# domanovi/FEC_Erasure_Code_Unit_Test_Relay

Measured on AMD Instinct MI355X. Metric: GiB/s device-resident erasure encode+decode, 300B pkts, T=10; %HBM roofline, higher is better.
Workload: dtype u8; 1 GPU; encode 1000010 + decode 1000000 x 300B packets per GPU, one stream per GPU, (T,B,N)=(10,3,3); T=10, B=3, N=3, packets_per_gpu=1000000

## Files before the change

### fec_erasure_code_unit_test_relay_amd/_lib.py

```python
from __future__ import annotations

import ctypes
import os

_HERE = os.path.dirname(os.path.abspath(__file__))
LIB_PATH = os.environ.get("FEC_AMD_LIB") or os.path.join(_HERE, "libfec_amd.so")
HEADER_PATHS = [os.path.join(_HERE, "..", "include", "fec_amd.h")]

FEC_OK = 0
FEC_ERR_ARG = -1
FEC_ERR_HIP = -2
FEC_ERR_NOMEM = -3
FEC_ERR_WORKSPACE = -4
FEC_ERR_SEQUENCE = -5
FEC_ERR_HISTORY = -6

KERNEL_NAMES = ["fec_encode_kernel", "fec_scan_kernel", "fec_plan_kernel", "fec_copy_kernel",
                "fec_recover_kernel"]


class FecError(RuntimeError):
    def __init__(self, status: int, what: str = ""):
        msg = lib().fec_strerror(status).decode() if _lib is not None else str(status)
        if status == FEC_ERR_HIP and _lib is not None:
# ... 4 lines not shown
        self.status = status


_lib = None


def lib() -> ctypes.CDLL:
    global _lib
    if _lib is not None:
        return _lib
    if not os.path.exists(LIB_PATH):
        raise RuntimeError(
            f"{LIB_PATH} is missing: the HIP extension must be built first "
            "(make -C fec_erasure_code_unit_test_relay_amd/csrc); there is no fallback")
    try:
        import torch
    except ImportError:
        pass
    L = ctypes.CDLL(LIB_PATH)
    vp, i32, i64 = ctypes.c_void_p, ctypes.c_int, ctypes.c_int64
    ip = ctypes.POINTER(ctypes.c_int)
    i64p = ctypes.POINTER(ctypes.c_int64)
    L.fec_strerror.restype = ctypes.c_char_p
    L.fec_strerror.argtypes = [i32]
    L.fec_last_error.restype = i32
    L.fec_last_error.argtypes = [ctypes.c_char_p, ctypes.c_size_t]
    L.fec_version.restype = i32
    L.fec_codec_create.argtypes = [i32, i32, i32, i32, ctypes.POINTER(vp)]
    L.fec_codec_destroy.argtypes = [vp]
    L.fec_codec_geometry.argtypes = [vp, ip, ip, ip, ip]
    L.fec_codec_generator.argtypes = [vp, vp]
    L.fec_codec_set_encode_path.argtypes = [vp, i32]
    L.fec_encode_tile_fetch.argtypes = [i32, i32, i32, i32, i32, ip, ip, ip, ip]
    L.fec_codec_set_copy_path.argtypes = [vp, i32]
    L.fec_codec_set_plan_path.argtypes = [vp, i32]
    L.fec_codec_info.argtypes = [vp, ctypes.c_char_p, ctypes.c_size_t]
    L.fec_codec_set_episode_dedup.argtypes = [vp, i32]
    L.fec_debug_stamps.argtypes = [vp, i32, vp]
    L.fec_encode_batch.argtypes = [vp, vp, vp, i64, i64, vp, vp, vp]
    L.fec_decode_workspace_bytes.restype = ctypes.c_size_t
    L.fec_decode_workspace_bytes.argtypes = [vp, i64]
    L.fec_decode_batch.argtypes = [vp, vp, vp, i64, vp, vp, vp, ctypes.c_size_t, vp]
    L.fec_decode_counters.argtypes = [vp, i64p, i64p, i64p]
    L.fec_streams_create.argtypes = [i32, i32, i32, i32, i32, ctypes.POINTER(vp)]
    L.fec_streams_destroy.argtypes = [vp]
    L.fec_streams_encode.argtypes = [vp, vp, i32, vp, vp, vp, vp, vp]
    L.fec_streams_decode.argtypes = [vp, vp, i32, vp, vp, vp, vp, vp]
    L.fec_streams_state.argtypes = [vp, i32, i64p, i64p]
    L.fec_streams_encode_burst.argtypes = [vp, vp, vp, i32, vp, vp, vp, vp, vp]
    L.fec_streams_decode_burst.argtypes = [vp, vp, vp, i32, vp, vp, vp, vp, vp]
    L.fec_streams_plan_burst_host.argtypes = [i32, i32, i32, i32, vp, vp, i32, vp]
    L.fec_streams_create_mixed.argtypes = [i32, vp, i32, vp, i32, ctypes.POINTER(vp)]
    L.fec_streams_codes.argtypes = [vp, ip, ip]
    L.fec_streams_stream_geometry.argtypes = [vp, i32, ip, ip, ip, ip, ip, ip]
    L.fec_streams_set_code.argtypes = [vp, i32, i32]
    L.fec_streams_mixed_fit.argtypes = [i32, vp, i32, vp, vp, vp, vp]
    L.fec_decode_stream_create.argtypes = [ctypes.POINTER(vp)]
    L.fec_decode_stream_destroy.argtypes = [vp]
    L.fec_decode_stream_state.argtypes = [vp, i64p, i64p]
    L.fec_decode_stream_push.argtypes = [vp, vp, vp, vp, vp, i64, i64, vp, vp, i64p, vp, ctypes.c_size_t, vp]
    L.fec_decode_plan_stats.argtypes = [vp, i64p, i64p]
    L.fec_decode_plan.argtypes = [vp, vp, i64, vp, ctypes.c_size_t, vp]
    L.fec_decode_apply.argtypes = [vp, vp, vp, i64, vp, vp, vp, ctypes.c_size_t, vp]
    L.fec_decode_copy.argtypes = [vp, vp, vp, i64, vp, vp, vp]
    L.fec_decode_recover.argtypes = [vp, vp, i64, vp, vp, vp, ctypes.c_size_t, vp]
    L.fec_timing_enable.argtypes = [vp, i32]
# ... 45 lines not shown
    L.fec_relay_streams_plan_host.argtypes = [i32, i32, vp, vp, i32, vp, vp]
    L.fec_sdswdf_create.argtypes = [i32, i32, i32, i32, i32, i32, ctypes.POINTER(vp)]
    L.fec_sdswdf_destroy.argtypes = [vp]
    L.fec_sdswdf_geometry.argtypes = [vp, ip, ip, ip, ip, ip, ip, ip]
    L.fec_sdswdf_tile_geometry.argtypes = [i32, i32, i32, i32, i32, i32, i64, ip, ip]
    L.fec_sdswdf_relay_batch.argtypes = [vp, vp, i64, vp, i64, vp, vp]
    L.fec_sdswdf_destination_batch.argtypes = [vp, vp, vp, i64, vp, vp, vp]
    L.fec_sdswdf_relay_plan.argtypes = [vp, vp, i64, vp, vp, i64, i64p, ip]
    L.fec_sdswdf_dest_plan.argtypes = [vp, vp, vp, i64, vp, vp, vp, i64, i64p, ip]
    L.fec_sdswdf_relay_batch_starts.argtypes = [vp, vp, i64, vp, i64, vp, i32, vp, vp]
    L.fec_sdswdf_destination_batch_starts.argtypes = [vp, vp, vp, i64, vp, i32, vp, vp, vp]
    L.fec_relay_vr_create.argtypes = [i32, i32, vp, i32, i64, ctypes.POINTER(vp)]
    L.fec_relay_vr_destroy.argtypes = [vp]
    L.fec_relay_vr_geometry.argtypes = [vp, ip, ip, ip]
    L.fec_relay_vr_run.argtypes = [vp, vp, vp, vp, vp, vp, vp, vp, vp]
    L.fec_relay_session_create.argtypes = [i32, i32, i64, vp, i64, vp, i64, ctypes.POINTER(vp)]
    L.fec_relay_session_destroy.argtypes = [vp]
    L.fec_relay_session_info.argtypes = [vp, vp, vp]
    L.fec_relay_session_relay_offsets.argtypes = [vp, vp]
    L.fec_relay_session_hop1_headers.argtypes = [vp, vp]
    L.fec_relay_session_dest_meta.argtypes = [vp, vp, vp]
    L.fec_relay_session_run.argtypes = [vp, vp, vp, vp, vp, vp, vp]
    L.fec_relay_session_hop1.argtypes = [vp, vp, i64, vp, vp]
    for name in ["fec_relay_session_create", "fec_relay_session_destroy", "fec_relay_session_info",
                 "fec_relay_session_relay_offsets", "fec_relay_session_hop1_headers", "fec_relay_session_dest_meta",
                 "fec_relay_session_run", "fec_relay_session_hop1", "fec_sdswdf_create", "fec_sdswdf_destroy", "fec_sdswdf_geometry", "fec_sdswdf_tile_geometry", "fec_sdswdf_relay_batch",
                 "fec_sdswdf_destination_batch", "fec_sdswdf_relay_plan", "fec_sdswdf_dest_plan",
                 "fec_sdswdf_relay_batch_starts", "fec_sdswdf_destination_batch_starts", "fec_relay_vr_create",
                 "fec_relay_vr_destroy", "fec_relay_vr_geometry", "fec_relay_vr_run",
                 "fec_swdf_create", "fec_swdf_destroy", "fec_swdf_geometry", "fec_swdf_relay_batch",
                 "fec_swdf_destination_batch", "fec_relay_streams_create", "fec_relay_streams_destroy",
                 "fec_relay_streams_geometry", "fec_relay_streams_relay", "fec_relay_streams_destination",
                 "fec_relay_streams_state", "fec_relay_streams_fit", "fec_relay_streams_plan_host", "fec_codec_create", "fec_codec_destroy", "fec_codec_set_encode_path",
                 "fec_encode_tile_fetch", "fec_codec_set_copy_path", "fec_codec_set_plan_path", "fec_codec_info", "fec_codec_set_episode_dedup", "fec_debug_stamps", "fec_codec_geometry",
                 "fec_codec_generator", "fec_encode_batch", "fec_decode_batch", "fec_decode_plan",
                 "fec_decode_stream_create", "fec_decode_stream_destroy", "fec_decode_stream_state",
                 "fec_decode_stream_push", "fec_streams_create", "fec_streams_destroy", "fec_streams_encode",
                 "fec_streams_decode", "fec_streams_state", "fec_streams_encode_burst",
                 "fec_streams_decode_burst", "fec_streams_plan_burst_host", "fec_streams_create_mixed",
                 "fec_streams_codes", "fec_streams_stream_geometry", "fec_streams_set_code",
                 "fec_streams_mixed_fit",
                 "fec_decode_apply", "fec_decode_copy", "fec_decode_recover",
                 "fec_decode_counters", "fec_decode_plan_stats", "fec_timing_enable", "fec_timing_collect",
                 "fec_encoder_create", "fec_encoder_destroy", "fec_encoder_transmit",
                 "fec_decoder_create", "fec_decoder_destroy", "fec_decoder_receive",
                 "fec_plan_host", "fec_util_fill_payload", "fec_erasure_iid",
                 "fec_erasure_three_sections_iid", "fec_erasure_ge", "fec_erasure_ge_varying",
                 "fec_erasure_fritchman_varying", "fec_erasure_periodic", "fec_vr_plan_create",
                 "fec_vr_plan_rerun", "fec_vr_plan_destroy", "fec_vr_plan_stats", "fec_vr_plan_timing", "fec_vr_plan_instances", "fec_vr_plan_packets",
                 "fec_vr_encode_batch", "fec_vr_decode_batch", "fec_vr_frames_batch", "fec_vr_parse_batch",
                 "fec_vr_plan_layout", "fec_vr_plan_row_offsets", "fec_block_encode_batch",
                 "fec_block_decode_batch"]:
        getattr(L, name).restype = i32
    _lib = L
    return _lib


def check(status: int, what: str) -> None:
    if status != FEC_OK:
        raise FecError(status, what)
```

### fec_erasure_code_unit_test_relay_amd/csrc/fec_codec.hip

```cpp
#include <hip/hip_runtime.h>
#include <hip/hip_ext.h>

#include <algorithm>
#include <atomic>
#include <chrono>
#include <functional>
#include <cstdio>
#include <cstdlib>
#include <cstring>
#include <memory>
#include <mutex>
#include <new>
#include <vector>

#include "fec_amd.h"
#include "fec_host.h"
#include "fec_kernels.h"
#include "fec_status.h"

using fec::Geometry;

namespace {

constexpr int kLdsBudget = 64 * 1024;
constexpr int kCopyLdsBudget = 32 * 1024;
constexpr int kMaxPayload = 1500;

inline int round16(int v) { return (v + 15) & ~15; }

#define HIP_TRY(expr)                                  \
    do {                                               \
        if ((expr) != hipSuccess) return FEC_ERR_HIP;  \
    } while (0)

struct EventPair {
    int kernel;
    hipEvent_t a, b;
};

}

struct fec_decode_stream {
    int64_t consumed = 0;
    int64_t last_cut = 0;
};

struct fec_codec {
    Geometry g;
// ... 128 lines not shown
            break;
        }
    for (int tp = 64; tp >= 1; tp >>= 1)
        if (c->copy_lds(tp) <= kLdsBudget) {
            c->copy_tp = tp;
            break;
        }
    if (!c->enc_tp || !c->copy_tp) return FEC_ERR_ARG;
    {
        int dev = 0;
        HIP_TRY(hipGetDevice(&dev));
        HIP_TRY(hipDeviceGetAttribute(&c->cus, hipDeviceAttributeMultiprocessorCount, dev));
    }
    if ((g.L & 3) == 0 && g.n - g.k >= 0) {
        const fec::TileGeom tg = fec::tile_geometry(g.k, g.n - g.k, g.L);
        if (tg.ok) c->tile_kernel = fec::fec_encode_tile_kernel_for(g.k, g.n - g.k, g.L);
        if (c->tile_kernel) {
            c->tile = tg;
            HIP_TRY(hipFuncSetAttribute(c->tile_kernel, hipFuncAttributeMaxDynamicSharedMemorySize, tg.lds_len));
            int per_cu = 0;
            HIP_TRY(hipOccupancyMaxActiveBlocksPerMultiprocessor(&per_cu, c->tile_kernel, 256, tg.lds));
            c->tile_per_cu = per_cu;
            if (per_cu <= 0) c->tile_kernel = nullptr;
        }
    }
    if ((g.L & 3) == 0) c->copy_fast = fec::fec_copy_fast_kernel_for(g.k, g.n - g.k);
    if (c->copy_fast)
        for (int tp = 64; tp >= 8; tp >>= 1)
            if (c->copyf_lds(tp) <= (tp == 8 ? kLdsBudget : kCopyLdsBudget)) {
                c->copyf_tp = tp;
                break;
            }
    if (!c->copyf_tp) c->copy_fast = nullptr;
    HIP_TRY(hipStreamCreateWithFlags(&c->side, hipStreamNonBlocking));
    HIP_TRY(hipEventCreateWithFlags(&c->ev_fork, hipEventDisableTiming));
    HIP_TRY(hipEventCreateWithFlags(&c->ev_join, hipEventDisableTiming));
    return FEC_OK;
}

struct WsLayout {
    size_t counters, erased, src_d, rec_list, sym_ok, coef, work, dups, keys, reps_tr, total;
    int tbits;
};

WsLayout ws_layout(const Geometry& g, int64_t P) {
    auto up = [](size_t v) { return (v + 255) & ~size_t(255); };
    WsLayout w;
    w.counters = 0;
    w.erased = up(64);
    w.src_d = w.erased + up(static_cast<size_t>(P) * 4);
    w.rec_list = w.src_d + up(static_cast<size_t>(P) * 4);
    w.sym_ok = w.rec_list + up(static_cast<size_t>(P) * 8);
    w.coef = w.sym_ok + up(static_cast<size_t>(P) * g.k);
    const size_t maxep = static_cast<size_t>(P) / static_cast<size_t>(g.T + 2) + 2;
    w.tbits = 8;
    while ((size_t(1) << w.tbits) < 2 * maxep) ++w.tbits;
    w.work = w.coef + up(static_cast<size_t>(P) * g.k * g.n);
    w.dups = w.work + up(maxep * 4);
    w.keys = w.dups + up(maxep * 8);
    w.reps_tr = w.keys + up((size_t(1) << w.tbits) * 8);
    w.total = w.reps_tr + up((size_t(1) << w.tbits) * 4);
    return w;
}

struct Ws {
    int32_t* counters;
// ... 259 lines not shown
    if (int st = check_ws(c, P, d_ws, ws_bytes)) return st;
    const Ws w = ws_carve(g, P, d_ws);
    fec::CompactArgs ca;
    ca.counters = w.counters;
    ca.erased = w.erased;
    ca.src_d = w.src_d;
    ca.sym_ok = w.sym_ok;
    ca.k = g.k;
    ca.rec_list = w.rec_list;
    if (!c->compact_fresh)
        HIP_TRY(hipMemsetAsync(w.counters + 2, 0, 4, s));
    c->compact_fresh = false;
    hipLaunchKernelGGL(fec::fec_compact_kernel, dim3(256), dim3(256), 0, s, ca);
    HIP_TRY(hipGetLastError());
    return FEC_OK;
}

int launch_recover(fec_codec* c, const uint8_t* d_cw, int64_t P, uint8_t* d_out, int32_t* d_outlen,
                   void* d_ws, size_t ws_bytes, hipStream_t s, int64_t row_off = 0, bool compacted = false) {
    const Geometry& g = c->g;
    const int64_t Pout = P - g.T;
    if (Pout <= 0) return FEC_OK;
    if (int st = check_ws(c, P, d_ws, ws_bytes)) return st;
    if (!compacted)
        if (int st = launch_compact(c, P, d_ws, ws_bytes, s)) return st;
    const Ws w = ws_carve(g, P, d_ws);
    fec::RecArgs ra;
    ra.cw = d_cw;
    ra.P = P;
    ra.Pout = Pout;
    ra.counters = w.counters;
    ra.rec_list = w.rec_list;
    ra.coef = w.coef;
    ra.gf = c->d_gf;
    ra.out = d_out;
    ra.out_len = d_outlen;
    ra.L = g.L;
    ra.k = g.k;
    ra.n = g.n;
    ra.S = g.S;
    ra.CW = g.CW;
    hipEvent_t stop;
    if (int st = c->begin(FEC_KERNEL_DEC_RECOVER, s, &stop)) return st;
    ra.row_off = row_off;
    ra.stamps = (c->stamp_kernel == FEC_KERNEL_DEC_RECOVER) ? c->d_stamps : nullptr;
    const int span = (g.k + g.n - 1) * g.CW + 32;
    ra.stage_bytes = (span <= 12 * 1024 && g.n <= 17) ? ((span + 15) & ~15) : 0;
    const unsigned rgrid = static_cast<unsigned>(std::min<int64_t>((Pout + 3) / 4, 1024));
    const int maxn = g.n <= 17 ? 17 : 32;
    const int lds = fec::recover_lds_bytes(maxn, ra.stage_bytes);
    if (g.n > 17)
        hipLaunchKernelGGL((fec::fec_recover_kernel_t<32, false>), dim3(rgrid), dim3(256), lds, s, ra);
    else if (ra.stage_bytes)
        hipLaunchKernelGGL((fec::fec_recover_kernel_t<17, true>), dim3(rgrid), dim3(256), lds, s, ra);
    else
        hipLaunchKernelGGL((fec::fec_recover_kernel_t<17, false>), dim3(rgrid), dim3(256), lds, s, ra);
    HIP_TRY(hipGetLastError());
    return c->end(stop, s);
}

int launch_decode(fec_codec* c, const uint8_t* d_cw, const uint8_t* d_er, int64_t P, uint8_t* d_out,
                  int32_t* d_outlen, void* d_ws, size_t ws_bytes, hipStream_t s) {
    if (P - c->g.T <= 0) return FEC_OK;
    if (int st = check_ws(c, P, d_ws, ws_bytes)) return st;
    HIP_TRY(hipEventRecord(c->ev_fork, s));
    HIP_TRY(hipStreamWaitEvent(c->side, c->ev_fork, 0));
    if (int st = launch_plan(c, d_er, P, d_ws, ws_bytes, c->side)) return st;
    if (int st = launch_compact(c, P, d_ws, ws_bytes, c->side)) return st;
    HIP_TRY(hipEventRecord(c->ev_join, c->side));
    if (int st = launch_copy(c, d_cw, d_er, P, d_out, d_outlen, s)) return st;
    HIP_TRY(hipStreamWaitEvent(s, c->ev_join, 0));
    return launch_recover(c, d_cw, P, d_out, d_outlen, d_ws, ws_bytes, s, 0, true);
}

int launch_decode_stream(fec_codec* c, fec_decode_stream* st, const uint8_t* d_cw, const uint8_t* d_er,
                         const uint8_t* h_er, int64_t P, int64_t history, uint8_t* d_out, int32_t* d_outlen,
                         int64_t* n_out, void* d_ws, size_t ws_bytes, hipStream_t s) {
    const int T = c->g.T;
    const int64_t s0 = st->consumed;
    const int64_t next_out = std::max<int64_t>(0, s0 - T);
    const int64_t end = s0 + P;
    const int64_t avail = s0 - history;
    *n_out = 0;
    if (P < 0 || history < 0 || avail < 0) return FEC_ERR_ARG;
    if (end - T <= next_out) {
        st->consumed = end;
        return FEC_OK;
    }
    if (s0 - next_out > history) return FEC_ERR_HISTORY;
// ... 362 lines not shown
    if (!c || path < 0 || path > 2) return FEC_ERR_ARG;
    if (path == 2 && !c->copy_fast) return FEC_ERR_ARG;
    c->copy_path = path;
    return FEC_OK;
}

int fec_codec_set_encode_path(fec_codec* c, int path) {
    if (!c || !(path == 0 || path == 1 || path == 5)) return FEC_ERR_ARG;
    if (path == 5 && !c->tile_kernel) return FEC_ERR_ARG;
    c->encode_path = path;
    return FEC_OK;
}

int fec_encode_tile_fetch(int max_payload, int T, int B, int N, int seg, int* R, int* issued, int* live_body,
                          int* live_front) {
    if (max_payload < 0 || T < 0 || B < 0 || N < 0 || N > T) return FEC_ERR_ARG;
    const int L = max_payload, k = T - N + 1, np = B, n = k + np;
    const fec::TileGeom tg = fec::tile_geometry(k, np, L, seg != 0);
    const bool have = (L & 3) == 0 && tg.ok &&
                      (seg ? fec::fec_encode_tile_seg_kernel_for(k, np, L) : fec::fec_encode_tile_kernel_for(k, np, L));
    int body = 0, front = 0;
    if (have) {
        const int CPR = (L + 15) >> 4;
        for (int c = 0; c < tg.ngl * 256; ++c) {
            body += fec::tile_piece_live(tg.R, CPR, n, c, false);
            front += np > 0 && fec::tile_piece_live(tg.R, CPR, n, c, true);
        }
    }
    if (R) *R = have ? tg.R : 0;
    if (issued) *issued = have ? tg.ngl * 256 : 0;
    if (live_body) *live_body = body;
    if (live_front) *live_front = front;
    return have ? 1 : 0;
}

int fec_timing_enable(fec_codec* c, int enable) {
    if (!c) return FEC_ERR_ARG;
    c->timing = enable != 0;
    return FEC_OK;
}

int fec_timing_collect(fec_codec* c, double* total_ms, int64_t* launches) {
    if (!c || !total_ms || !launches) return FEC_ERR_ARG;
    for (int i = 0; i < FEC_KERNEL_COUNT; ++i) {
        total_ms[i] = 0.0;
        launches[i] = 0;
    }
    for (auto& e : c->events) {
        HIP_TRY(hipEventSynchronize(e.b));
        float ms = 0.f;
        HIP_TRY(hipEventElapsedTime(&ms, e.a, e.b));
        total_ms[e.kernel] += ms;
        launches[e.kernel] += 1;
        (void)hipEventDestroy(e.a);
        (void)hipEventDestroy(e.b);
    }
    c->events.clear();
    return FEC_OK;
}

namespace {
hipError_t host_mapped(uint8_t** host, uint8_t** dev, size_t bytes) {
    if (hipError_t e = hipHostMalloc(reinterpret_cast<void**>(host), bytes,
                                     hipHostMallocMapped | hipHostMallocCoherent))
        return e;
    std::memset(*host, 0, bytes);
// ... 586 lines not shown
```

### fec_erasure_code_unit_test_relay_amd/csrc/fec_kernels.h

```cpp
#pragma once

#include <hip/hip_runtime.h>
#include <cstddef>
#include <stdint.h>

namespace fec {

struct EncArgs {
    const uint8_t* payload;
    const int32_t* len;
    int64_t history;
    int64_t P;
    uint8_t* cw;
    int32_t* cw_len;
    const uint32_t* ptab;
    int L, k, n, S, CW;
    int SP;
    int TP;
    int ROWS;
    int plane;
    int xin_bytes, xout_bytes;
};

struct TileGeom {
// ... 159 lines not shown
struct EpisodeArgs {
    const uint8_t* er;
    int64_t P, Pout;
    int T;
    int tbits;
    int dedup;
    int32_t* counters;
    int32_t* erased;
    int32_t* src_d;
    int32_t* work;
    int32_t* dups;
    uint64_t* keys;
    int32_t* reps_tr;
    uint64_t* stamps;
};
__global__ void fec_episode_kernel(EpisodeArgs a);

struct CompactArgs {
    int32_t* counters;
    const int32_t* erased;
    const int32_t* src_d;
    const uint8_t* sym_ok;
    int k;
    int32_t* rec_list;
};
__global__ void fec_compact_kernel(CompactArgs a);

struct RecArgs {
    const uint8_t* cw;
    int64_t P, Pout;
    const int32_t* counters;
    const int32_t* rec_list;
    const uint8_t* coef;
    const uint8_t* gf;
    uint8_t* out;
    int32_t* out_len;
    int L, k, n, S, CW;
    int64_t row_off;
    int stage_bytes;
    uint64_t* stamps;
};
inline int recover_lds_bytes(int maxn, int stage_bytes) {
    return 1552 + 4 * (((2 * 16 * maxn + 15) & ~15) + stage_bytes);
}
template <int MAXN, bool STAGED>
__global__ void fec_recover_kernel_t(RecArgs a);


struct BlockArgs {
    const uint8_t* in;
    const uint8_t* er;
    uint8_t* out;
    uint8_t* er_out;
    int64_t nblk;
    int k, n;
    const uint8_t* G;
    const uint8_t* gf;
    const uint8_t* rules;
    int64_t wbase_n;
    int ES;
};
__global__ void fec_block_encode_kernel(BlockArgs a);

struct CodecView {
    int L, T, B, N, k, n, S, CW;
    const uint8_t* G;
    const uint8_t* gf;
    const uint8_t* rules;
    int64_t wbase_n;
    int ES;
    const uint32_t* ptab;
};
__global__ void fec_block_decode_kernel(BlockArgs a);

__global__ void fec_encode_kernel(EncArgs a);
__global__ void fec_plan_kernel(PlanArgs a);
__global__ void fec_copy_kernel(CopyArgs a);

// ... 55 lines not shown
```

### fec_erasure_code_unit_test_relay_amd/csrc/fec_kernels.hip

```cpp
#include "fec_device.h"
#include "fec_kernels.h"

namespace fec {

__device__ __forceinline__ uint32_t gf_mul4(const uint32_t* tab, uint32_t x) {
    const uint32_t g0 = x & 0x07070707u;
    const uint32_t g1 = (x >> 3) & 0x07070707u;
    const uint32_t g2 = (x >> 6) & 0x03030303u;
    return __builtin_amdgcn_perm(tab[1], tab[0], g0) ^ __builtin_amdgcn_perm(tab[3], tab[2], g1) ^
           __builtin_amdgcn_perm(tab[4], tab[4], g2);
}

__device__ __forceinline__ uint8_t gf_mul_lds(const uint8_t* gexp, const uint8_t* glog, uint8_t a,
                                              uint8_t b) {
    return (a && b) ? gexp[glog[a] + glog[b]] : 0;
}

__global__ __launch_bounds__(256) void fec_encode_kernel(EncArgs a) {
    extern __shared__ __attribute__((aligned(16))) uint8_t smem[];
    uint8_t* xin = smem;
    uint8_t* xout = smem + a.xin_bytes;
    uint16_t* hmap = reinterpret_cast<uint16_t*>(xout + a.xout_bytes);
    const int Sk = a.S * a.k;
    int32_t* rowlen = reinterpret_cast<int32_t*>(hmap + ((Sk + 7) & ~7));

    const int tid = threadIdx.x;
    const int k = a.k, n = a.n, S = a.S, L = a.L, SP = a.SP, H = n - 1;
    const int64_t t0 = static_cast<int64_t>(blockIdx.x) * a.TP;
    const int ntile = static_cast<int>(min<int64_t>(a.TP, a.P - t0));
    const int rows = ntile + H;

    for (int o = tid * 16; o < a.xin_bytes; o += 256 * 16)
        *reinterpret_cast<uint4*>(xin + o) = make_uint4(0, 0, 0, 0);
    for (int h = tid; h < Sk; h += 256) hmap[h] = static_cast<uint16_t>((h % k) * a.plane + h / k);
// ... 346 lines not shown
    const int ner = a.counters[1];
    const int J = 64 / k;
    const int jl = lane / k, il = lane - jl * k;
    const int waves = gridDim.x * (blockDim.x >> 6);
    for (int r0 = (blockIdx.x * (blockDim.x >> 6) + (threadIdx.x >> 6)) * J; r0 < ner; r0 += waves * J) {
        const int r = r0 + jl;
        const bool valid = jl < J && r < ner;
        int x = 0, xr = 0;
        bool bad = false;
        if (valid) {
            x = a.erased[r];
            xr = x + a.src_d[x];
            bad = !a.sym_ok[static_cast<int64_t>(xr) * k + il];
        }
        const uint64_t badm = __builtin_amdgcn_ballot_w64(bad);
        const bool lead = valid && il == 0;
        uint64_t gbad = 0;
        for (int s = 0; s < k; ++s) gbad |= badm >> s;
        const bool ok = lead && !((gbad >> lane) & 1u);
        const uint64_t okm = __builtin_amdgcn_ballot_w64(ok);
        if (okm) {
            int base = 0;
            if (lane == __builtin_ctzll(okm)) base = atomicAdd(&a.counters[2], __builtin_popcountll(okm));
            base = __shfl(base, __builtin_ctzll(okm));
            if (ok) {
                const int at = base + __builtin_popcountll(okm & ((1ull << lane) - 1ull));
                a.rec_list[2 * at] = x;
                a.rec_list[2 * at + 1] = xr;
            }
        }
    }
}

constexpr int kRecMaxK = 16;
constexpr int kRecLogZero = 512;
constexpr int kRecStageChunks = 12;

template <int MAXN, bool STAGED>
__global__ __launch_bounds__(256) void fec_recover_kernel_t(RecArgs a) {
    extern __shared__ __attribute__((aligned(16))) uint8_t rsm[];
    uint8_t* ex = rsm;
    uint16_t* lg = reinterpret_cast<uint16_t*>(rsm + 1040);
    const int tid = threadIdx.x;
    const int lane = tid & 63, wl = tid >> 6;
    const int L = a.L, k = a.k, n = a.n, CW = a.CW;
    constexpr int kLcBytes = (2 * kRecMaxK * MAXN + 15) & ~15;
    uint16_t* lc = reinterpret_cast<uint16_t*>(rsm + 1552 + wl * (kLcBytes + a.stage_bytes));
    uint8_t* rows = rsm + 1552 + wl * (kLcBytes + a.stage_bytes) + kLcBytes;
    phase_stamp(a.stamps, blockIdx.x, 0);
    for (int i = tid; i < 1040; i += 256) ex[i] = i < 512 ? a.gf[i] : 0;
    for (int i = tid; i < 256; i += 256) lg[i] = i ? a.gf[512 + i] : static_cast<uint16_t>(kRecLogZero);
    __syncthreads();
    phase_stamp(a.stamps, blockIdx.x, 1);
    const int nrec = a.counters[2];
    const int waves = gridDim.x * 4;
    const int64_t cw_total = a.P * CW;
    {
        for (int r = blockIdx.x * 4 + wl; r < nrec; r += waves) {
            const int x = a.rec_list[2 * r], xr = a.rec_list[2 * r + 1];
            if (x < a.row_off) continue;
            uint8_t* orow = a.out + static_cast<int64_t>(x - a.row_off) * L;
            const int rlo = x - k + 1 > 0 ? x - k + 1 : 0;
            const int64_t s0 = static_cast<int64_t>(rlo) * CW;
            const int64_t s1 = static_cast<int64_t>(x + n < a.P ? x + n : a.P) * CW;
            const int64_t a0 = s0 & ~int64_t(15);
            uint4 piece[STAGED ? kRecStageChunks : 1];
            const int nb = STAGED ? static_cast<int>((s1 - a0 + 15) >> 4) : 0;
            if constexpr (STAGED) {
#pragma unroll
                for (int j = 0; j < kRecStageChunks; ++j) {
                    const int c = lane + 64 * j;
                    const int64_t o = a0 + 16 * c;
                    piece[j] = make_uint4(0u, 0u, 0u, 0u);
                    if (c < nb) {
                        if (o + 16 <= cw_total) {
                            piece[j] = *reinterpret_cast<const uint4*>(a.cw + o);
                        } else {
                            uint32_t t[4] = {0u, 0u, 0u, 0u};
                            for (int e = 0; e < 16; ++e)
                                if (o + e < cw_total) t[e >> 2] |= static_cast<uint32_t>(a.cw[o + e]) << (8 * (e & 3));
                            piece[j] = make_uint4(t[0], t[1], t[2], t[3]);
                        }
                    }
                }
            }
            constexpr int kCf = (kRecMaxK * MAXN + 63) / 64;
            uint32_t cf[kCf];
            const uint8_t* cfp = a.coef + static_cast<int64_t>(xr) * k * n;
#pragma unroll
            for (int j = 0; j < kCf; ++j) cf[j] = lane + 64 * j < k * n ? cfp[lane + 64 * j] : 0u;
            if constexpr (STAGED) {
#pragma unroll
                for (int j = 0; j < kRecStageChunks; ++j)
                    if (lane + 64 * j < nb) *reinterpret_cast<uint4*>(rows + 16 * (lane + 64 * j)) = piece[j];
            }
#pragma unroll
            for (int j = 0; j < kCf; ++j)
                if (lane + 64 * j < k * n) lc[lane + 64 * j] = lg[cf[j]];
            __builtin_amdgcn_fence(__ATOMIC_RELEASE, "wavefront");
            __builtin_amdgcn_wave_barrier();
            __builtin_amdgcn_fence(__ATOMIC_ACQUIRE, "wavefront");
            int ln = 0;
            for (int h0 = 0; h0 < L + 2; h0 += 64) {
                const int h = h0 + lane;
                const int sidx = h / k, i = h - sidx * k;
                const int qlo = i - x > 0 ? i - x : 0;
                const int qhi = h < L + 2 ? min(n, static_cast<int>(a.P - x) + i) : 0;
                const int base = (x - i - rlo) * CW + static_cast<int>(s0 - a0) + sidx * n;
                uint32_t lq[MAXN], v[MAXN];
#pragma unroll
                for (int q = 0; q < MAXN; ++q) {
                    const bool use = q >= qlo && q < qhi;
                    lq[q] = lc[i * n + (q < n ? q : 0)];
                    if constexpr (STAGED) {
                        v[q] = use ? rows[base + q * (CW + 1)] : 0u;
                    } else {
                        v[q] = use ? a.cw[static_cast<int64_t>(x - i + q) * CW + sidx * n + q] : 0u;
                    }
                }
                uint32_t acc = 0;
#pragma unroll
                for (int q = 0; q < MAXN; ++q) acc ^= ex[lq[q] + lg[v[q]]];
                if (h0 == 0) {
                    const int hi = __builtin_amdgcn_readlane(static_cast<int>(acc), 0);
                    const int lo = __builtin_amdgcn_readlane(static_cast<int>(acc), 1);
                    ln = min(hi * 256 + lo, L);
                }
                const int b = h - 2;
                if (b >= 0 && b < L) orow[b] = b < ln ? static_cast<uint8_t>(acc) : 0;
            }
            if (lane == 0) a.out_len[x - a.row_off] = ln;
            __builtin_amdgcn_wave_barrier();
        }
    }
    phase_stamp(a.stamps, blockIdx.x, 2);
}

template __global__ void fec_recover_kernel_t<17, true>(RecArgs);
template __global__ void fec_recover_kernel_t<17, false>(RecArgs);
template __global__ void fec_recover_kernel_t<32, false>(RecArgs);

__global__ __launch_bounds__(256) void fec_copy_kernel(CopyArgs a) {
    extern __shared__ __attribute__((aligned(16))) uint8_t smem[];
    uint8_t* cwt = smem;
    uint16_t* omap = reinterpret_cast<uint16_t*>(smem + a.cwt_bytes);
    int32_t* clen = reinterpret_cast<int32_t*>(omap + ((a.L + 2 + 7) & ~7));
    const int tid = threadIdx.x;
    const int L = a.L, k = a.k, n = a.n, CW = a.CW;
    const int64_t x0 = static_cast<int64_t>(blockIdx.x) * a.TP;
    const int ntile = static_cast<int>(min<int64_t>(a.TP, a.Pout - x0));

    for (int h = tid; h < L + 2; h += 256) omap[h] = static_cast<uint16_t>((h / k) * n + h % k);
    const int bytes = ntile * CW;
    const uint8_t* src = a.cw + x0 * CW;
    if ((bytes & 15) == 0 && (reinterpret_cast<uintptr_t>(src) & 15) == 0) {
        for (int o = tid * 16; o < bytes; o += 256 * 16)
            *reinterpret_cast<uint4*>(cwt + o) = *reinterpret_cast<const uint4*>(src + o);
    } else {
        for (int o = tid; o < bytes; o += 256) cwt[o] = src[o];
    }
    __syncthreads();
    for (int tl = tid; tl < ntile; tl += 256) {
        const int64_t x = x0 + tl;
        int ln = 0, copy = 0;
        if (!a.er[x]) {
            const uint8_t* row = cwt + tl * CW;
            const int hdr = row[omap[0]] * 256 + row[omap[1]];
            bool slow = false;
            for (int d = 0; d <= a.T; ++d) slow = slow || a.er[x + d];
            ln = slow ? min(hdr, L) : hdr;
            copy = min(ln, L);
        }
        clen[tl] = copy;
// ... 52 lines not shown
```

### include/fec_amd.h

```cpp
#ifndef FEC_AMD_H
#define FEC_AMD_H

#include <stddef.h>
#include <stdint.h>

#ifdef __cplusplus
extern "C" {
#endif

#define FEC_OK 0
#define FEC_ERR_ARG (-1)
#define FEC_ERR_HIP (-2)
#define FEC_ERR_NOMEM (-3)
#define FEC_ERR_WORKSPACE (-4)
#define FEC_ERR_SEQUENCE (-5)
#define FEC_ERR_HISTORY (-6)

typedef struct fec_codec fec_codec;
typedef struct fec_encoder fec_encoder;
typedef struct fec_decoder fec_decoder;

#define FEC_AMD_ABI_VERSION 2

const char *fec_strerror(int status);
int fec_last_error(char *buf, size_t size);
int fec_version(void);

int fec_codec_create(int max_payload, int T, int B, int N, fec_codec **out);
int fec_codec_destroy(fec_codec *codec);
int fec_codec_geometry(const fec_codec *codec, int *k, int *n, int *S, int *CW);
int fec_codec_info(const fec_codec *codec, char *buf, size_t size);
int fec_codec_set_encode_path(fec_codec *codec, int path);
int fec_encode_tile_fetch(int max_payload, int T, int B, int N, int seg, int *R, int *issued, int *live_body,
                          int *live_front);
int fec_codec_set_copy_path(fec_codec *codec, int path);
int fec_codec_set_plan_path(fec_codec *codec, int path);
int fec_codec_set_episode_dedup(fec_codec *codec, int on);
int fec_codec_generator(const fec_codec *codec, uint8_t *G);

int fec_encode_batch(fec_codec *codec, const uint8_t *d_payload, const int32_t *d_payload_len,
                     int64_t history, int64_t P, uint8_t *d_codeword, int32_t *d_codeword_len,
                     void *hip_stream);

size_t fec_decode_workspace_bytes(const fec_codec *codec, int64_t P);
int fec_decode_batch(fec_codec *codec, const uint8_t *d_codeword, const uint8_t *d_erasure,
                     int64_t P, uint8_t *d_payload_out, int32_t *d_payload_len, void *d_workspace,
                     size_t workspace_bytes, void *hip_stream);
typedef struct fec_decode_stream fec_decode_stream;
int fec_decode_stream_create(fec_decode_stream **out);
int fec_decode_stream_destroy(fec_decode_stream *st);
int fec_decode_stream_push(fec_codec *codec, fec_decode_stream *st, const uint8_t *d_codeword,
                           const uint8_t *d_erasure, const uint8_t *h_erasure, int64_t P, int64_t history,
                           uint8_t *d_payload_out, int32_t *d_payload_len, int64_t *n_out,
                           void *d_workspace, size_t workspace_bytes, void *hip_stream);
int fec_decode_stream_state(const fec_decode_stream *st, int64_t *consumed, int64_t *last_cut);
int fec_decode_plan(fec_codec *codec, const uint8_t *d_erasure, int64_t P, void *d_workspace,
                    size_t workspace_bytes, void *hip_stream);
int fec_decode_apply(fec_codec *codec, const uint8_t *d_codeword, const uint8_t *d_erasure,
                     int64_t P, uint8_t *d_payload_out, int32_t *d_payload_len, void *d_workspace,
                     size_t workspace_bytes, void *hip_stream);
int fec_decode_copy(fec_codec *codec, const uint8_t *d_codeword, const uint8_t *d_erasure,
                    int64_t P, uint8_t *d_payload_out, int32_t *d_payload_len, void *hip_stream);
int fec_decode_recover(fec_codec *codec, const uint8_t *d_codeword, int64_t P,
                       uint8_t *d_payload_out, int32_t *d_payload_len, void *d_workspace,
                       size_t workspace_bytes, void *hip_stream);
int fec_decode_counters(const void *d_workspace, int64_t *episodes, int64_t *recovered,
                        int64_t *lost);
// ... 183 lines not shown
```

Baseline: 967.6 GiB/s.

## Replace log/exp table GF recovery with packed bit-plane GF(2^8) arithmetic

The recover kernel no longer does GF multiplication through log/exp lookup tables held in LDS. It precomputes per-coefficient bit masks and computes four output bytes per lane with packed 32-bit bit-plane XOR accumulation, folding with xtime reduction at the end. Small rows are split across lane groups that combine results with shuffles, the next rec_list entry is prefetched, outputs are written as dwords, and the template no longer depends on MAXN. LDS sizing is now computed per geometry. The cost is more ALU work per term and more LDS spent on masks, in exchange for removing the dependent table lookups and the table load at block start.

```diff
diff --git a/fec_erasure_code_unit_test_relay_amd/_lib.py b/fec_erasure_code_unit_test_relay_amd/_lib.py
--- a/fec_erasure_code_unit_test_relay_amd/_lib.py
+++ b/fec_erasure_code_unit_test_relay_amd/_lib.py
@@ -60,6 +60,7 @@
     L.fec_codec_generator.argtypes = [vp, vp]
     L.fec_codec_set_encode_path.argtypes = [vp, i32]
     L.fec_encode_tile_fetch.argtypes = [i32, i32, i32, i32, i32, ip, ip, ip, ip]
+    L.fec_gf_dot4_host.argtypes = [vp, vp, i32, vp]
     L.fec_codec_set_copy_path.argtypes = [vp, i32]
     L.fec_codec_set_plan_path.argtypes = [vp, i32]
     L.fec_codec_info.argtypes = [vp, ctypes.c_char_p, ctypes.c_size_t]
@@ -171,7 +172,7 @@
                  "fec_swdf_destination_batch", "fec_relay_streams_create", "fec_relay_streams_destroy",
                  "fec_relay_streams_geometry", "fec_relay_streams_relay", "fec_relay_streams_destination",
                  "fec_relay_streams_state", "fec_relay_streams_fit", "fec_relay_streams_plan_host", "fec_codec_create", "fec_codec_destroy", "fec_codec_set_encode_path",
-                 "fec_encode_tile_fetch", "fec_codec_set_copy_path", "fec_codec_set_plan_path", "fec_codec_info", "fec_codec_set_episode_dedup", "fec_debug_stamps", "fec_codec_geometry",
+                 "fec_encode_tile_fetch", "fec_gf_dot4_host", "fec_codec_set_copy_path", "fec_codec_set_plan_path", "fec_codec_info", "fec_codec_set_episode_dedup", "fec_debug_stamps", "fec_codec_geometry",
                  "fec_codec_generator", "fec_encode_batch", "fec_decode_batch", "fec_decode_plan",
                  "fec_decode_stream_create", "fec_decode_stream_destroy", "fec_decode_stream_state",
                  "fec_decode_stream_push", "fec_streams_create", "fec_streams_destroy", "fec_streams_encode",
diff --git a/fec_erasure_code_unit_test_relay_amd/csrc/fec_codec.hip b/fec_erasure_code_unit_test_relay_amd/csrc/fec_codec.hip
--- a/fec_erasure_code_unit_test_relay_amd/csrc/fec_codec.hip
+++ b/fec_erasure_code_unit_test_relay_amd/csrc/fec_codec.hip
@@ -14,6 +14,7 @@
 #include <vector>
 
 #include "fec_amd.h"
+#include "fec_gf_packed.h"
 #include "fec_host.h"
 #include "fec_kernels.h"
 #include "fec_status.h"
@@ -208,6 +209,13 @@
                 break;
             }
     if (!c->copyf_tp) c->copy_fast = nullptr;
+    {
+        fec::RecArgs ra;
+        const int lds = fec::recover_lds(g.k, g.n, g.CW, &ra);
+        const void* rk = ra.stage_bytes ? reinterpret_cast<const void*>(&fec::fec_recover_kernel_t<true>)
+                                        : reinterpret_cast<const void*>(&fec::fec_recover_kernel_t<false>);
+        if (lds > 64 * 1024) HIP_TRY(hipFuncSetAttribute(rk, hipFuncAttributeMaxDynamicSharedMemorySize, lds));
+    }
     HIP_TRY(hipStreamCreateWithFlags(&c->side, hipStreamNonBlocking));
     HIP_TRY(hipEventCreateWithFlags(&c->ev_fork, hipEventDisableTiming));
     HIP_TRY(hipEventCreateWithFlags(&c->ev_join, hipEventDisableTiming));
@@ -533,7 +541,6 @@
     ra.counters = w.counters;
     ra.rec_list = w.rec_list;
     ra.coef = w.coef;
-    ra.gf = c->d_gf;
     ra.out = d_out;
     ra.out_len = d_outlen;
     ra.L = g.L;
@@ -545,17 +552,13 @@
     if (int st = c->begin(FEC_KERNEL_DEC_RECOVER, s, &stop)) return st;
     ra.row_off = row_off;
     ra.stamps = (c->stamp_kernel == FEC_KERNEL_DEC_RECOVER) ? c->d_stamps : nullptr;
-    const int span = (g.k + g.n - 1) * g.CW + 32;
-    ra.stage_bytes = (span <= 12 * 1024 && g.n <= 17) ? ((span + 15) & ~15) : 0;
-    const unsigned rgrid = static_cast<unsigned>(std::min<int64_t>((Pout + 3) / 4, 1024));
-    const int maxn = g.n <= 17 ? 17 : 32;
-    const int lds = fec::recover_lds_bytes(maxn, ra.stage_bytes);
-    if (g.n > 17)
-        hipLaunchKernelGGL((fec::fec_recover_kernel_t<32, false>), dim3(rgrid), dim3(256), lds, s, ra);
-    else if (ra.stage_bytes)
-        hipLaunchKernelGGL((fec::fec_recover_kernel_t<17, true>), dim3(rgrid), dim3(256), lds, s, ra);
+    const int lds = fec::recover_lds(g.k, g.n, g.CW, &ra);
+    constexpr int W = fec::kRecWaves;
+    const unsigned rgrid = static_cast<unsigned>(std::min<int64_t>((Pout + W - 1) / W, 4096 / W));
+    if (ra.stage_bytes)
+        hipLaunchKernelGGL((fec::fec_recover_kernel_t<true>), dim3(rgrid), dim3(64 * W), lds, s, ra);
     else
-        hipLaunchKernelGGL((fec::fec_recover_kernel_t<17, false>), dim3(rgrid), dim3(256), lds, s, ra);
+        hipLaunchKernelGGL((fec::fec_recover_kernel_t<false>), dim3(rgrid), dim3(64 * W), lds, s, ra);
     HIP_TRY(hipGetLastError());
     return c->end(stop, s);
 }
@@ -984,6 +987,12 @@
     if (live_body) *live_body = body;
     if (live_front) *live_front = front;
     return have ? 1 : 0;
+}
+
+int fec_gf_dot4_host(const uint32_t* coef4, const uint32_t* data4, int nterms, uint32_t* out4) {
+    if (nterms < 0 || (nterms > 0 && (!coef4 || !data4)) || !out4) return FEC_ERR_ARG;
+    *out4 = fec::gf4_dot(coef4, data4, nterms);
+    return FEC_OK;
 }
 
 int fec_timing_enable(fec_codec* c, int enable) {
diff --git a/fec_erasure_code_unit_test_relay_amd/csrc/fec_gf_packed.h b/fec_erasure_code_unit_test_relay_amd/csrc/fec_gf_packed.h
--- /dev/null
+++ b/fec_erasure_code_unit_test_relay_amd/csrc/fec_gf_packed.h
@@ -0,0 +1,48 @@
+#pragma once
+
+#include <stdint.h>
+
+#if defined(__HIPCC__) || defined(__CUDACC__)
+#define FEC_GF_HD __host__ __device__ __forceinline__
+#else
+#define FEC_GF_HD inline
+#endif
+
+namespace fec {
+
+FEC_GF_HD void gf4_coef_masks(uint32_t c, uint32_t m[8]) {
+#pragma unroll
+    for (int b = 0; b < 8; ++b) {
+        const uint32_t t = (c >> b) & 0x01010101u;
+        m[b] = (t << 8) - t;
+    }
+}
+
+FEC_GF_HD void gf4_accumulate(uint32_t plane[8], const uint32_t m[8], uint32_t v) {
+#pragma unroll
+    for (int b = 0; b < 8; ++b) plane[b] ^= m[b] & v;
+}
+
+FEC_GF_HD uint32_t gf4_xtime(uint32_t a) {
+    const uint32_t hi = (a >> 7) & 0x01010101u;
+    return ((a & 0x7f7f7f7fu) << 1) ^ ((hi << 4) | (hi << 3) | (hi << 2) | hi);
+}
+
+FEC_GF_HD uint32_t gf4_fold(const uint32_t plane[8]) {
+    uint32_t r = plane[7];
+#pragma unroll
+    for (int b = 6; b >= 0; --b) r = gf4_xtime(r) ^ plane[b];
+    return r;
+}
+
+FEC_GF_HD uint32_t gf4_dot(const uint32_t* coef4, const uint32_t* data4, int nterms) {
+    uint32_t plane[8] = {0, 0, 0, 0, 0, 0, 0, 0};
+    for (int t = 0; t < nterms; ++t) {
+        uint32_t m[8];
+        gf4_coef_masks(coef4[t], m);
+        gf4_accumulate(plane, m, data4[t]);
+    }
+    return gf4_fold(plane);
+}
+
+}
diff --git a/fec_erasure_code_unit_test_relay_amd/csrc/fec_kernels.h b/fec_erasure_code_unit_test_relay_amd/csrc/fec_kernels.h
--- a/fec_erasure_code_unit_test_relay_amd/csrc/fec_kernels.h
+++ b/fec_erasure_code_unit_test_relay_amd/csrc/fec_kernels.h
@@ -215,18 +215,23 @@
     const int32_t* counters;
     const int32_t* rec_list;
     const uint8_t* coef;
-    const uint8_t* gf;
     uint8_t* out;
     int32_t* out_len;
     int L, k, n, S, CW;
     int64_t row_off;
-    int stage_bytes;
+    int mask_bytes, coef_bytes, stage_bytes, wave_bytes;
     uint64_t* stamps;
 };
-inline int recover_lds_bytes(int maxn, int stage_bytes) {
-    return 1552 + 4 * (((2 * 16 * maxn + 15) & ~15) + stage_bytes);
-}
-template <int MAXN, bool STAGED>
+constexpr int kRecWaves = 4;
+inline int recover_lds(int k, int n, int CW, RecArgs* a) {
+    const int span = (k + n - 1) * CW + 32;
+    a->mask_bytes = k * n * 32;
+    a->coef_bytes = (k * n + 15) & ~15;
+    a->stage_bytes = span <= 12 * 1024 ? ((span + 15) & ~15) : 0;
+    a->wave_bytes = a->mask_bytes + a->coef_bytes + a->stage_bytes;
+    return kRecWaves * a->wave_bytes;
+}
+template <bool STAGED>
 __global__ void fec_recover_kernel_t(RecArgs a);
 
 
diff --git a/fec_erasure_code_unit_test_relay_amd/csrc/fec_kernels.hip b/fec_erasure_code_unit_test_relay_amd/csrc/fec_kernels.hip
--- a/fec_erasure_code_unit_test_relay_amd/csrc/fec_kernels.hip
+++ b/fec_erasure_code_unit_test_relay_amd/csrc/fec_kernels.hip
@@ -1,5 +1,8 @@
 #include "fec_device.h"
+#include "fec_gf_packed.h"
 #include "fec_kernels.h"
+
+#include <type_traits>
 
 namespace fec {
 
@@ -412,113 +415,190 @@
     }
 }
 
-constexpr int kRecMaxK = 16;
-constexpr int kRecLogZero = 512;
 constexpr int kRecStageChunks = 12;
-
-template <int MAXN, bool STAGED>
+constexpr int kRecCoefLoads = (16 * 32 + 63) / 64;
+
+template <bool STAGED, bool EDGE>
+__device__ __forceinline__ uint32_t recover_dword(const uint8_t* src, int64_t origin, const uint32_t* mk, int m,
+                                                  int x, int64_t P, int L, int k, int n, int CW, int q0,
+                                                  int qstep) {
+    using off_t = typename std::conditional<STAGED, int, int64_t>::type;
+    const int H = 4 * m + 2 + 2 * k;
+    int s = H / k, i = H - s * k;
+    s -= 2;
+    const uint32_t* mrow = mk + i * n * 8;
+    off_t base[4];
+    int qlo[4], qhi[4];
+#pragma unroll
+    for (int j = 0; j < 4; ++j) {
+        const int h = 4 * m + 2 + j;
+        const bool valid = h >= 0 && h < L + 2;
+        const int sj = valid ? s : 0, ij = valid ? i : 0;
+        base[j] = static_cast<off_t>(static_cast<int64_t>(x - ij) * CW + sj * n - origin);
+        qlo[j] = ij - x > 0 ? ij - x : 0;
+        qhi[j] = static_cast<int>(min<int64_t>(n, P - x + ij));
+        if (++i == k) {
+            i = 0;
+            ++s;
+        }
+    }
+    uint32_t plane[8] = {0, 0, 0, 0, 0, 0, 0, 0};
+#pragma unroll 4
+    for (int q = q0; q < n; q += qstep) {
+        uint32_t v = 0;
+#pragma unroll
+        for (int j = 0; j < 4; ++j) {
+            const off_t o = base[j] + q * (CW + 1);
+            uint32_t byte;
+            if constexpr (EDGE) {
+                const bool use = q >= qlo[j] && q < qhi[j];
+                byte = src[use ? o : off_t(0)];
+                byte = use ? byte : 0u;
+            } else {
+                byte = src[o];
+            }
+            v |= byte << (8 * j);
+        }
+        const uint4 m0 = *reinterpret_cast<const uint4*>(mrow + q * 8);
+        const uint4 m1 = *reinterpret_cast<const uint4*>(mrow + q * 8 + 4);
+        const uint32_t mm[8] = {m0.x, m0.y, m0.z, m0.w, m1.x, m1.y, m1.z, m1.w};
+        gf4_accumulate(plane, mm, v);
+    }
+    return gf4_fold(plane);
+}
+
+template <bool STAGED>
 __global__ __launch_bounds__(256) void fec_recover_kernel_t(RecArgs a) {
     extern __shared__ __attribute__((aligned(16))) uint8_t rsm[];
-    uint8_t* ex = rsm;
-    uint16_t* lg = reinterpret_cast<uint16_t*>(rsm + 1040);
     const int tid = threadIdx.x;
     const int lane = tid & 63, wl = tid >> 6;
-    const int L = a.L, k = a.k, n = a.n, CW = a.CW;
-    constexpr int kLcBytes = (2 * kRecMaxK * MAXN + 15) & ~15;
-    uint16_t* lc = reinterpret_cast<uint16_t*>(rsm + 1552 + wl * (kLcBytes + a.stage_bytes));
-    uint8_t* rows = rsm + 1552 + wl * (kLcBytes + a.stage_bytes) + kLcBytes;
+    const int L = a.L, k = a.k, n = a.n, CW = a.CW, kn = a.k * a.n;
+    uint8_t* wave_lds = rsm + wl * a.wave_bytes;
+    uint32_t* mk = reinterpret_cast<uint32_t*>(wave_lds);
+    uint8_t* cfb = wave_lds + a.mask_bytes;
+    uint8_t* rows = cfb + a.coef_bytes;
     phase_stamp(a.stamps, blockIdx.x, 0);
-    for (int i = tid; i < 1040; i += 256) ex[i] = i < 512 ? a.gf[i] : 0;
-    for (int i = tid; i < 256; i += 256) lg[i] = i ? a.gf[512 + i] : static_cast<uint16_t>(kRecLogZero);
-    __syncthreads();
+    const int wpw = blockDim.x >> 6;
+    const int waves = gridDim.x * wpw;
+    int r = blockIdx.x * wpw + wl;
+    int2 ent = make_int2(0, 0);
+    if (r < a.Pout) ent = *reinterpret_cast<const int2*>(a.rec_list + 2 * r);
+    const int nrec = a.counters[2];
     phase_stamp(a.stamps, blockIdx.x, 1);
-    const int nrec = a.counters[2];
-    const int waves = gridDim.x * 4;
     const int64_t cw_total = a.P * CW;
-    {
-        for (int r = blockIdx.x * 4 + wl; r < nrec; r += waves) {
-            const int x = a.rec_list[2 * r], xr = a.rec_list[2 * r + 1];
-            if (x < a.row_off) continue;
-            uint8_t* orow = a.out + static_cast<int64_t>(x - a.row_off) * L;
-            const int rlo = x - k + 1 > 0 ? x - k + 1 : 0;
-            const int64_t s0 = static_cast<int64_t>(rlo) * CW;
-            const int64_t s1 = static_cast<int64_t>(x + n < a.P ? x + n : a.P) * CW;
-            const int64_t a0 = s0 & ~int64_t(15);
-            uint4 piece[STAGED ? kRecStageChunks : 1];
-            const int nb = STAGED ? static_cast<int>((s1 - a0 + 15) >> 4) : 0;
-            if constexpr (STAGED) {
-#pragma unroll
-                for (int j = 0; j < kRecStageChunks; ++j) {
-                    const int c = lane + 64 * j;
-                    const int64_t o = a0 + 16 * c;
-                    piece[j] = make_uint4(0u, 0u, 0u, 0u);
-                    if (c < nb) {
-                        if (o + 16 <= cw_total) {
-                            piece[j] = *reinterpret_cast<const uint4*>(a.cw + o);
-                        } else {
-                            uint32_t t[4] = {0u, 0u, 0u, 0u};
-                            for (int e = 0; e < 16; ++e)
-                                if (o + e < cw_total) t[e >> 2] |= static_cast<uint32_t>(a.cw[o + e]) << (8 * (e & 3));
-                            piece[j] = make_uint4(t[0], t[1], t[2], t[3]);
-                        }
+    bool first = true;
+    while (r < nrec) {
+        const int x = ent.x, xr = ent.y;
+        const int rnext = r + waves;
+        if (rnext < nrec) ent = *reinterpret_cast<const int2*>(a.rec_list + 2 * rnext);
+        r = rnext;
+        if (x < a.row_off) continue;
+        uint8_t* orow = a.out + static_cast<int64_t>(x - a.row_off) * L;
+        const int rlo = x - k + 1 > 0 ? x - k + 1 : 0;
+        const int64_t s0 = static_cast<int64_t>(rlo) * CW;
+        const int64_t s1 = static_cast<int64_t>(x + n < a.P ? x + n : a.P) * CW;
+        const int64_t a0 = s0 & ~int64_t(15);
+        uint8_t cf[kRecCoefLoads];
+        const uint8_t* cfp = a.coef + static_cast<int64_t>(xr) * kn;
+#pragma unroll
+        for (int j = 0; j < kRecCoefLoads; ++j) cf[j] = lane + 64 * j < kn ? cfp[lane + 64 * j] : uint8_t(0);
+        uint4 piece[STAGED ? kRecStageChunks : 1];
+        const int nb = STAGED ? static_cast<int>((s1 - a0 + 15) >> 4) : 0;
+        if constexpr (STAGED) {
+#pragma unroll
+            for (int j = 0; j < kRecStageChunks; ++j) {
+                const int c = lane + 64 * j;
+                const int64_t o = a0 + 16 * c;
+                piece[j] = make_uint4(0u, 0u, 0u, 0u);
+                if (c < nb) {
+                    if (o + 16 <= cw_total) {
+                        piece[j] = *reinterpret_cast<const uint4*>(a.cw + o);
+                    } else {
+                        uint32_t t[4] = {0u, 0u, 0u, 0u};
+                        for (int e = 0; e < 16; ++e)
+                            if (o + e < cw_total) t[e >> 2] |= static_cast<uint32_t>(a.cw[o + e]) << (8 * (e & 3));
+                        piece[j] = make_uint4(t[0], t[1], t[2], t[3]);
                     }
                 }
             }
-            constexpr int kCf = (kRecMaxK * MAXN + 63) / 64;
-            uint32_t cf[kCf];
-            const uint8_t* cfp = a.coef + static_cast<int64_t>(xr) * k * n;
-#pragma unroll
-            for (int j = 0; j < kCf; ++j) cf[j] = lane + 64 * j < k * n ? cfp[lane + 64 * j] : 0u;
-            if constexpr (STAGED) {
-#pragma unroll
-                for (int j = 0; j < kRecStageChunks; ++j)
-                    if (lane + 64 * j < nb) *reinterpret_cast<uint4*>(rows + 16 * (lane + 64 * j)) = piece[j];
-            }
-#pragma unroll
-            for (int j = 0; j < kCf; ++j)
-                if (lane + 64 * j < k * n) lc[lane + 64 * j] = lg[cf[j]];
-            __builtin_amdgcn_fence(__ATOMIC_RELEASE, "wavefront");
-            __builtin_amdgcn_wave_barrier();
-            __builtin_amdgcn_fence(__ATOMIC_ACQUIRE, "wavefront");
-            int ln = 0;
-            for (int h0 = 0; h0 < L + 2; h0 += 64) {
-                const int h = h0 + lane;
-                const int sidx = h / k, i = h - sidx * k;
-                const int qlo = i - x > 0 ? i - x : 0;
-                const int qhi = h < L + 2 ? min(n, static_cast<int>(a.P - x) + i) : 0;
-                const int base = (x - i - rlo) * CW + static_cast<int>(s0 - a0) + sidx * n;
-                uint32_t lq[MAXN], v[MAXN];
-#pragma unroll
-                for (int q = 0; q < MAXN; ++q) {
-                    const bool use = q >= qlo && q < qhi;
-                    lq[q] = lc[i * n + (q < n ? q : 0)];
-                    if constexpr (STAGED) {
-                        v[q] = use ? rows[base + q * (CW + 1)] : 0u;
-                    } else {
-                        v[q] = use ? a.cw[static_cast<int64_t>(x - i + q) * CW + sidx * n + q] : 0u;
-                    }
+        }
+#pragma unroll
+        for (int j = 0; j < kRecCoefLoads; ++j)
+            if (lane + 64 * j < kn) cfb[lane + 64 * j] = cf[j];
+        __builtin_amdgcn_fence(__ATOMIC_RELEASE, "wavefront");
+        __builtin_amdgcn_wave_barrier();
+        __builtin_amdgcn_fence(__ATOMIC_ACQUIRE, "wavefront");
+        for (int e = lane; e < kn; e += 64) {
+            const int i0 = e / n, q = e - i0 * n;
+            uint32_t c4 = 0;
+            int ii = i0;
+#pragma unroll
+            for (int j = 0; j < 4; ++j) {
+                c4 |= static_cast<uint32_t>(cfb[ii * n + q]) << (8 * j);
+                if (++ii == k) ii = 0;
+            }
+            uint32_t mm[8];
+            gf4_coef_masks(c4, mm);
+            *reinterpret_cast<uint4*>(mk + e * 8) = make_uint4(mm[0], mm[1], mm[2], mm[3]);
+            *reinterpret_cast<uint4*>(mk + e * 8 + 4) = make_uint4(mm[4], mm[5], mm[6], mm[7]);
+        }
+        if constexpr (STAGED) {
+#pragma unroll
+            for (int j = 0; j < kRecStageChunks; ++j)
+                if (lane + 64 * j < nb) *reinterpret_cast<uint4*>(rows + 16 * (lane + 64 * j)) = piece[j];
+        }
+        __builtin_amdgcn_fence(__ATOMIC_RELEASE, "wavefront");
+        __builtin_amdgcn_wave_barrier();
+        __builtin_amdgcn_fence(__ATOMIC_ACQUIRE, "wavefront");
+        if (first) phase_stamp(a.stamps, blockIdx.x, 2);
+        const uint8_t* src = STAGED ? rows : a.cw;
+        const int64_t origin = STAGED ? a0 : 0;
+        const bool edge = x < k - 1 || x + n > a.P;
+        const bool dwords = (reinterpret_cast<uintptr_t>(orow) & 3) == 0;
+        const int nitem = (L + 3) / 4 + 1;
+        int ln = 0;
+        for (int it0 = 0; it0 < nitem; it0 += 64) {
+            const int left = nitem - it0;
+            int gs = 0;
+            while (gs < 3 && (left << (gs + 1)) <= 64) ++gs;
+            const int G = 1 << gs, g = lane & (G - 1);
+            const int m = it0 + (lane >> gs) - 1;
+            const bool act = (lane >> gs) < left;
+            uint32_t acc = 0;
+            if (act) {
+                if (edge)
+                    acc = recover_dword<STAGED, true>(src, origin, mk, m, x, a.P, L, k, n, CW, g, G);
+                else if (gs == 0)
+                    acc = recover_dword<STAGED, false>(src, origin, mk, m, x, a.P, L, k, n, CW, 0, 1);
+                else
+                    acc = recover_dword<STAGED, false>(src, origin, mk, m, x, a.P, L, k, n, CW, g, G);
+            }
+            for (int o = 1; o < G; o <<= 1) acc ^= static_cast<uint32_t>(__shfl_xor(static_cast<int>(acc), o));
+            if (it0 == 0) {
+                const uint32_t w = static_cast<uint32_t>(__builtin_amdgcn_readlane(static_cast<int>(acc), 0));
+                ln = min(static_cast<int>(((w >> 16) & 0xffu) * 256u + (w >> 24)), L);
+            }
+            if (act && g == 0 && m >= 0) {
+                const int b0 = 4 * m;
+                const int keep = min(max(ln - b0, 0), 4);
+                const uint32_t val = keep >= 4 ? acc : acc & ((1u << (8 * keep)) - 1u);
+                if (dwords && b0 + 4 <= L) {
+                    *reinterpret_cast<uint32_t*>(orow + b0) = val;
+                } else {
+                    for (int j = 0; j < 4 && b0 + j < L; ++j) orow[b0 + j] = static_cast<uint8_t>(val >> (8 * j));
                 }
-                uint32_t acc = 0;
-#pragma unroll
-                for (int q = 0; q < MAXN; ++q) acc ^= ex[lq[q] + lg[v[q]]];
-                if (h0 == 0) {
-                    const int hi = __builtin_amdgcn_readlane(static_cast<int>(acc), 0);
-                    const int lo = __builtin_amdgcn_readlane(static_cast<int>(acc), 1);
-                    ln = min(hi * 256 + lo, L);
-                }
-                const int b = h - 2;
-                if (b >= 0 && b < L) orow[b] = b < ln ? static_cast<uint8_t>(acc) : 0;
-            }
-            if (lane == 0) a.out_len[x - a.row_off] = ln;
-            __builtin_amdgcn_wave_barrier();
-        }
-    }
-    phase_stamp(a.stamps, blockIdx.x, 2);
-}
-
-template __global__ void fec_recover_kernel_t<17, true>(RecArgs);
-template __global__ void fec_recover_kernel_t<17, false>(RecArgs);
-template __global__ void fec_recover_kernel_t<32, false>(RecArgs);
+            }
+        }
+        if (lane == 0) a.out_len[x - a.row_off] = ln;
+        if (first) phase_stamp(a.stamps, blockIdx.x, 3);
+        first = false;
+        __builtin_amdgcn_wave_barrier();
+    }
+    phase_stamp(a.stamps, blockIdx.x, 4);
+}
+
+template __global__ void fec_recover_kernel_t<true>(RecArgs);
+template __global__ void fec_recover_kernel_t<false>(RecArgs);
 
 __global__ __launch_bounds__(256) void fec_copy_kernel(CopyArgs a) {
     extern __shared__ __attribute__((aligned(16))) uint8_t smem[];
diff --git a/include/fec_amd.h b/include/fec_amd.h
--- a/include/fec_amd.h
+++ b/include/fec_amd.h
@@ -33,6 +33,7 @@
 int fec_codec_set_encode_path(fec_codec *codec, int path);
 int fec_encode_tile_fetch(int max_payload, int T, int B, int N, int seg, int *R, int *issued, int *live_body,
                           int *live_front);
+int fec_gf_dot4_host(const uint32_t *coef4, const uint32_t *data4, int nterms, uint32_t *out4);
 int fec_codec_set_copy_path(fec_codec *codec, int path);
 int fec_codec_set_plan_path(fec_codec *codec, int path);
 int fec_codec_set_episode_dedup(fec_codec *codec, int on);
```

Measured after the change: 984.7 GiB/s, median of 3. Within noise of the previous version (+1.8%).
